# kritsanan1/Qwen3-TTS

Measured on AMD Instinct MI355X. Metric: audio-seconds/sec (RTF) + p50 first-packet latency, 1.7B @ batch 1/8, 1->8 GPU, higher is better.
Workload: dtype bf16; 1 GPU; Qwen3-TTS-12Hz-1.7b-customvoice B=8/GPU x 200-token prompts, streaming text, 256 frames + codec decode; global_batch=8, seq_len=200, frames=256, parallelism=dp1

## Files before the change

### qwen3-tts_amd/csrc/codec_unit.hip

```cpp
#include "common.h"

namespace {

constexpr int CU_TAPS = 7;
constexpr int CU_MAX_DIL = 9;

constexpr int unit_wpe(int C, int MI) { return C == 96 ? (MI == 4 ? 2 : 4) : (MI == 1 ? 3 : 2); }

template <int C, int MI>
__global__ __launch_bounds__(256) __attribute__((amdgpu_waves_per_eu(unit_wpe(C, MI)))) void codec_unit_k(
    qt_codec_resunit_args p) {
  constexpr int BM = 64 * MI;
  constexpr int RT = BM / 32;
  constexpr int NCH = C / 32;
  constexpr int CT = C / 32;
  constexpr int G = C / 8;
  constexpr int LDW = C + 8;
  constexpr int RPI = 256 / G;
  constexpr int NR = BM * G / 256;
  static_assert(BM * G % 256 == 0, "output tile groups divide over the block");
  extern __shared__ __attribute__((aligned(16))) unsigned char cu_smem[];
  bf16_t* img = (bf16_t*)cu_smem;
  const int tid = threadIdx.x, lane = tid & 63, w = tid >> 6;
  const int lm = lane & 15, lk = lane >> 4;
  const int dil = p.dil, halo = (CU_TAPS - 1) * dil, WR = BM + halo;
  const int tiles_t = (p.L + BM - 1) / BM;
  const int bi = blockIdx.x / tiles_t, t0 = (blockIdx.x - bi * tiles_t) * BM;
  const bf16_t* xin = (const bf16_t*)p.x_in + (long long)bi * p.L * C;
  bf16_t* xout = (bf16_t*)p.x_out + (long long)bi * p.L * C;

  {
    const int g = tid % G, r0 = tid / G;
    if (r0 < RPI) {
      float sa[8], sib[8];
      load8f(p.s1_alpha + g * 8, sa);
      load8f(p.s1_inv_beta + g * 8, sib);
      for (int rb = r0; rb < WR; rb += 4 * RPI) {
        u32x4_t raw[4];
#pragma unroll
        for (int u = 0; u < 4; ++u) {
          const int r = rb + u * RPI, ti = t0 - halo + r;
          raw[u] = u32x4_t{0u, 0u, 0u, 0u};
          if (r < WR && ti >= 0 && ti < p.L) raw[u] = *(const u32x4_t*)(xin + (long long)ti * C + g * 8);
        }
#pragma unroll
        for (int u = 0; u < 4; ++u) {
          const int r = rb + u * RPI;
          if (r >= WR) break;
          float v[8];
#pragma unroll
          for (int i = 0; i < 4; ++i) {
            v[2 * i] = __uint_as_float(raw[u][i] << 16);
            v[2 * i + 1] = __uint_as_float(raw[u][i] & 0xFFFF0000u);
          }
#pragma unroll
          for (int e = 0; e < 8; ++e) {
            const float sn = __sinf(v[e] * sa[e]);
            v[e] = v[e] + sib[e] * (sn * sn);
          }
          *(u32x4_t*)(img + r * LDW + g * 8) =
              u32x4_t{pack2bf(v[0], v[1]), pack2bf(v[2], v[3]), pack2bf(v[4], v[5]), pack2bf(v[6], v[7])};
        }
      }
    }
  }

  const int wrow = (w >> 1) * (BM / 2);
  const int nt0 = (w & 1) * CT;
  f32x4_t acc[RT][CT];
#pragma unroll
  for (int i = 0; i < RT; ++i)
#pragma unroll
    for (int q = 0; q < CT; ++q) acc[i][q] = f32x4_t{0.f, 0.f, 0.f, 0.f};

  {
    constexpr int KT = CU_TAPS * NCH;
    const bf16_t* Wb = (const bf16_t*)p.w1 + lane * 8;
    u32x4_t cur[CT], nxt[CT];
#pragma unroll
    for (int q = 0; q < CT; ++q) cur[q] = *(const u32x4_t*)(Wb + ((size_t)(nt0 + q) * KT) * 512);
    __syncthreads();
#pragma unroll 1
    for (int c = 0; c < NCH; ++c) {
      const bf16_t* wa = img + (wrow + lm) * LDW + c * 32 + lk * 8;
#pragma unroll
      for (int j = 0; j < CU_TAPS; ++j) {
        const int kn = j + 1 < CU_TAPS ? (j + 1) * NCH + c : (c + 1 < NCH ? c + 1 : c);
#pragma unroll
        for (int q = 0; q < CT; ++q) nxt[q] = *(const u32x4_t*)(Wb + ((size_t)(nt0 + q) * KT + kn) * 512);
        u32x4_t af[RT];
#pragma unroll
        for (int i = 0; i < RT; ++i) af[i] = *(const u32x4_t*)(wa + (i * 16 + j * dil) * LDW);
#pragma unroll
        for (int i = 0; i < RT; ++i)
#pragma unroll
          for (int q = 0; q < CT; ++q)
            acc[i][q] = __builtin_amdgcn_mfma_f32_16x16x32_bf16(__builtin_bit_cast(bf16x8_t, af[i]),
                                                                __builtin_bit_cast(bf16x8_t, cur[q]), acc[i][q], 0, 0, 0);
#pragma unroll
        for (int q = 0; q < CT; ++q) cur[q] = nxt[q];
      }
    }
  }
  __syncthreads();

  u32x4_t xr[NR];
#pragma unroll
  for (int u = 0; u < NR; ++u) {
    const int q = tid + u * 256, r = q / G, g = q - r * G;
    xr[u] = u32x4_t{0u, 0u, 0u, 0u};
    if (t0 + r < p.L) xr[u] = *(const u32x4_t*)(xin + (long long)(t0 + r) * C + g * 8);
  }

#pragma unroll
  for (int q = 0; q < CT; ++q) {
    const int n = (nt0 + q) * 16 + lm;
    const float b1 = p.b1 ? p.b1[n] : 0.f, a2 = p.s2_alpha[n], ib2 = p.s2_inv_beta[n];
#pragma unroll
    for (int i = 0; i < RT; ++i)
#pragma unroll
      for (int e = 0; e < 4; ++e) {
        const float h = bf2f(f2bf(acc[i][q][e] + b1));
        const float sn = __sinf(h * a2);
        img[(wrow + i * 16 + lk * 4 + e) * LDW + n] = f2bf(h + ib2 * (sn * sn));
        acc[i][q][e] = 0.f;
      }
  }

  {
    const bf16_t* Wb = (const bf16_t*)p.w2 + lane * 8;
    u32x4_t cur[CT], nxt[CT];
#pragma unroll
    for (int q = 0; q < CT; ++q) cur[q] = *(const u32x4_t*)(Wb + ((size_t)(nt0 + q) * NCH) * 512);
    __syncthreads();
    const bf16_t* wa = img + (wrow + lm) * LDW + lk * 8;
#pragma unroll
    for (int c = 0; c < NCH; ++c) {
      const int kn = c + 1 < NCH ? c + 1 : c;
#pragma unroll
      for (int q = 0; q < CT; ++q) nxt[q] = *(const u32x4_t*)(Wb + ((size_t)(nt0 + q) * NCH + kn) * 512);
      u32x4_t af[RT];
#pragma unroll
      for (int i = 0; i < RT; ++i) af[i] = *(const u32x4_t*)(wa + i * 16 * LDW + c * 32);
#pragma unroll
      for (int i = 0; i < RT; ++i)
#pragma unroll
        for (int q = 0; q < CT; ++q)
          acc[i][q] = __builtin_amdgcn_mfma_f32_16x16x32_bf16(__builtin_bit_cast(bf16x8_t, af[i]),
                                                              __builtin_bit_cast(bf16x8_t, cur[q]), acc[i][q], 0, 0, 0);
#pragma unroll
      for (int q = 0; q < CT; ++q) cur[q] = nxt[q];
    }
  }
  __syncthreads();

#pragma unroll
  for (int u = 0; u < NR; ++u) {
    const int q = tid + u * 256, r = q / G, g = q - r * G;
    *(u32x4_t*)(img + r * LDW + g * 8) = xr[u];
  }
  __syncthreads();
#pragma unroll
  for (int q = 0; q < CT; ++q) {
    const int n = (nt0 + q) * 16 + lm;
    const float b2 = p.b2 ? p.b2[n] : 0.f;
#pragma unroll
    for (int i = 0; i < RT; ++i)
#pragma unroll
      for (int e = 0; e < 4; ++e) {
        bf16_t* s = img + (wrow + i * 16 + lk * 4 + e) * LDW + n;
        *s = f2bf(bf2f(*s) + (acc[i][q][e] + b2));
      }
  }
  __syncthreads();

#pragma unroll
  for (int u = 0; u < NR; ++u) {
    const int q = tid + u * 256, r = q / G, g = q - r * G;
    if (t0 + r < p.L) *(u32x4_t*)(xout + (long long)(t0 + r) * C + g * 8) = *(const u32x4_t*)(img + r * LDW + g * 8);
  }
}

size_t unit_smem(int C, int bm, int dil) { return (size_t)(bm + (CU_TAPS - 1) * dil) * (C + 8) * sizeof(bf16_t); }

template <int C, int MI>
int launch_unit(const qt_codec_resunit_args& a, hipStream_t s) {
  constexpr int BM = 64 * MI;
  const size_t smem = unit_smem(C, BM, a.dil);
  if (smem > (64u << 10) &&
      hipFuncSetAttribute((const void*)codec_unit_k<C, MI>, hipFuncAttributeMaxDynamicSharedMemorySize,
                          (int)unit_smem(C, BM, CU_MAX_DIL)) != hipSuccess)
    return QT_ERR_LAUNCH;
  const long long blocks = (long long)a.B * ((a.L + BM - 1) / BM);
  hipLaunchKernelGGL((codec_unit_k<C, MI>), dim3((unsigned)blocks), dim3(256), smem, s, a);
  return hipGetLastError() == hipSuccess ? QT_OK : QT_ERR_LAUNCH;
}

}

static int unit_check(const qt_codec_resunit_args* a) {
  if (!a) return QT_ERR_ARG;
  if (a->a_dtype != QT_BF16 || a->w_dtype != QT_BF16) return QT_ERR_DTYPE;
  if (a->C != 96 && a->C != 192) return QT_ERR_SHAPE;
  if (a->dil != 1 && a->dil != 3 && a->dil != CU_MAX_DIL) return QT_ERR_SHAPE;
  if (a->B < 1 || a->L < 1 || (long long)a->B * ((a->L + 63) / 64) > 0x7FFFFFFFLL) return QT_ERR_SHAPE;
  if (!a->x_in || !a->x_out || !a->w1 || !a->w2 || !a->s1_alpha || !a->s1_inv_beta || !a->s2_alpha || !a->s2_inv_beta)
    return QT_ERR_ARG;
  if ((reinterpret_cast<uintptr_t>(a->x_in) | reinterpret_cast<uintptr_t>(a->x_out) | reinterpret_cast<uintptr_t>(a->w1) |
       reinterpret_cast<uintptr_t>(a->w2) | reinterpret_cast<uintptr_t>(a->s1_alpha) |
       reinterpret_cast<uintptr_t>(a->s1_inv_beta)) & 15)
    return QT_ERR_ARG;
  const unsigned long long bytes = (unsigned long long)a->B * a->L * a->C * sizeof(bf16_t);
  const uintptr_t xi = reinterpret_cast<uintptr_t>(a->x_in), xo = reinterpret_cast<uintptr_t>(a->x_out);
  if (xi < xo + bytes && xo < xi + bytes) return QT_ERR_ARG;
  return QT_OK;
}

extern "C" int qt_codec_resunit_supported(const qt_codec_resunit_args* a) { return unit_check(a) == QT_OK; }

extern "C" int qt_codec_resunit(const qt_codec_resunit_args* a, void* stream) {
  const int rc = unit_check(a);
  if (rc != QT_OK) return rc;
  hipStream_t s = (hipStream_t)stream;
  if constexpr (kProbe) {
    const int mi = qt_knob("QT_CU_MI", 0);
    if (a->C == 96 && mi == 1) return launch_unit<96, 1>(*a, s);
    if (a->C == 96 && mi == 4) return launch_unit<96, 4>(*a, s);
    if (a->C == 192 && (mi == 2 || mi == 4)) return launch_unit<192, 2>(*a, s);
  }
  if (a->C == 96) return launch_unit<96, 2>(*a, s);
  return launch_unit<192, 1>(*a, s);
}
```

Before: 251.4 audio-seconds/sec.

## Add fused wide-channel codec residual-unit kernel for C=384/768

Adds a new fused residual-unit kernel for codec decoder stages with 384 or 768 channels, which were previously rejected by the shape check and so fell back to another path. Input channels are streamed through a double-buffered shared-memory window in KC-sized chunks, with the snake activation applied on the fly, so the dilated 7-tap conv, the second snake, the 1x1 conv and the residual add all run in one kernel. This targets the separate launches and global-memory round trips the unfused path needs. In exchange it adds a large templated kernel with probe knobs and many MFMA accumulators per wave, which may increase register pressure.

```diff
diff --git a/qwen3-tts_amd/csrc/codec_unit.hip b/qwen3-tts_amd/csrc/codec_unit.hip
--- a/qwen3-tts_amd/csrc/codec_unit.hip
+++ b/qwen3-tts_amd/csrc/codec_unit.hip
@@ -196,12 +196,226 @@
   return hipGetLastError() == hipSuccess ? QT_OK : QT_ERR_LAUNCH;
 }
 
+constexpr int wide_threads(int C) { return 128 * (C / 96); }
+constexpr int WIDE_KC = 64, WIDE_RT = 4;
+
+constexpr size_t wide_img_bytes(int C, int KC, int dil) {
+  const size_t win = (size_t)2 * (64 + (CU_TAPS - 1) * dil) * (KC + 8) * sizeof(bf16_t);
+  const size_t at = (size_t)64 * (C + 8) * sizeof(bf16_t);
+  return win > at ? win : at;
+}
+constexpr size_t wide_smem(int C, int KC, int dil) { return wide_img_bytes(C, KC, dil) + (size_t)2 * C * sizeof(float); }
+
+template <int C, int KC, int RT>
+__global__ __launch_bounds__(wide_threads(C)) __attribute__((amdgpu_waves_per_eu(4))) void codec_unit_wide_k(
+    qt_codec_resunit_args p) {
+  constexpr int BM = 64;
+  constexpr int CT = 12 / RT;
+  constexpr int NTH = wide_threads(C);
+  constexpr int NWC = C / (16 * CT);
+  constexpr int NCH = C / 32;
+  constexpr int SUB = KC / 32;
+  constexpr int NCC = C / KC;
+  constexpr int G = C / 8;
+  constexpr int GK = KC / 8;
+  constexpr int LDW = C + 8;
+  constexpr int LDK = KC + 8;
+  constexpr int RPI = NTH / GK;
+  constexpr int NP = (BM + (CU_TAPS - 1) * CU_MAX_DIL + RPI - 1) / RPI;
+  constexpr int NR = BM * G / NTH;
+  static_assert((RT == 2 || RT == 4) && C % 96 == 0 && C % KC == 0 && KC % 32 == 0 && NTH % GK == 0 && BM * G % NTH == 0, "wide unit geometry");
+  extern __shared__ __attribute__((aligned(16))) unsigned char cu_smem[];
+  const int tid = threadIdx.x, lane = tid & 63, w = tid >> 6;
+  const int lm = lane & 15, lk = lane >> 4;
+  const int dil = p.dil, halo = (CU_TAPS - 1) * dil, WR = BM + halo;
+  bf16_t* img = (bf16_t*)cu_smem;
+  float* sn1 = (float*)(cu_smem + wide_img_bytes(C, KC, dil));
+  const int tiles_t = (p.L + BM - 1) / BM;
+  const int bi = blockIdx.x / tiles_t, t0 = (blockIdx.x - bi * tiles_t) * BM;
+  const bf16_t* xin = (const bf16_t*)p.x_in + (long long)bi * p.L * C;
+  bf16_t* xout = (bf16_t*)p.x_out + (long long)bi * p.L * C;
+
+  const int sg = tid % GK, sr0 = tid / GK;
+  u32x4_t raw[NP];
+  auto load_chunk = [&](int cc) {
+#pragma unroll
+    for (int u = 0; u < NP; ++u) {
+      const int r = sr0 + u * RPI, ti = t0 - halo + r;
+      raw[u] = u32x4_t{0u, 0u, 0u, 0u};
+      if (r < WR && ti >= 0 && ti < p.L) raw[u] = *(const u32x4_t*)(xin + (long long)ti * C + cc * KC + sg * 8);
+    }
+  };
+  auto store_chunk = [&](int buf, int cc) {
+    bf16_t* wb = img + (size_t)buf * WR * LDK;
+    float sa[8], sib[8];
+    load8f(sn1 + cc * KC + sg * 8, sa);
+    load8f(sn1 + C + cc * KC + sg * 8, sib);
+#pragma unroll
+    for (int u = 0; u < NP; ++u) {
+      const int r = sr0 + u * RPI;
+      if (r >= WR) break;
+      float v[8];
+#pragma unroll
+      for (int i = 0; i < 4; ++i) {
+        v[2 * i] = __uint_as_float(raw[u][i] << 16);
+        v[2 * i + 1] = __uint_as_float(raw[u][i] & 0xFFFF0000u);
+      }
+#pragma unroll
+      for (int e = 0; e < 8; ++e) {
+        const float sn = __sinf(v[e] * sa[e]);
+        v[e] = v[e] + sib[e] * (sn * sn);
+      }
+      *(u32x4_t*)(wb + r * LDK + sg * 8) =
+          u32x4_t{pack2bf(v[0], v[1]), pack2bf(v[2], v[3]), pack2bf(v[4], v[5]), pack2bf(v[6], v[7])};
+    }
+  };
+
+  load_chunk(0);
+  for (int i = tid; i < C; i += NTH) {
+    sn1[i] = p.s1_alpha[i];
+    sn1[C + i] = p.s1_inv_beta[i];
+  }
+  __syncthreads();
+  store_chunk(0, 0);
+
+  const int wrow = (w / NWC) * (16 * RT);
+  const int nt0 = (w % NWC) * CT;
+  f32x4_t acc[RT][CT];
+#pragma unroll
+  for (int i = 0; i < RT; ++i)
+#pragma unroll
+    for (int q = 0; q < CT; ++q) acc[i][q] = f32x4_t{0.f, 0.f, 0.f, 0.f};
+
+  {
+    constexpr int KT = CU_TAPS * NCH;
+    const bf16_t* Wb = (const bf16_t*)p.w1 + lane * 8;
+    u32x4_t cur[CT], nxt[CT];
+#pragma unroll
+    for (int q = 0; q < CT; ++q) cur[q] = *(const u32x4_t*)(Wb + ((size_t)(nt0 + q) * KT) * 512);
+    __syncthreads();
+#pragma unroll 1
+    for (int c = 0; c < NCH; ++c) {
+      const int cc = c / SUB, sub = c - cc * SUB;
+      if (sub == 0 && cc + 1 < NCC) load_chunk(cc + 1);
+      const bf16_t* wa = img + (size_t)(cc & 1) * WR * LDK + (wrow + lm) * LDK + sub * 32 + lk * 8;
+#pragma unroll
+      for (int j = 0; j < CU_TAPS; ++j) {
+        const int kn = j + 1 < CU_TAPS ? (j + 1) * NCH + c : (c + 1 < NCH ? c + 1 : c);
+#pragma unroll
+        for (int q = 0; q < CT; ++q) nxt[q] = *(const u32x4_t*)(Wb + ((size_t)(nt0 + q) * KT + kn) * 512);
+        u32x4_t af[RT];
+#pragma unroll
+        for (int i = 0; i < RT; ++i) af[i] = *(const u32x4_t*)(wa + (i * 16 + j * dil) * LDK);
+#pragma unroll
+        for (int i = 0; i < RT; ++i)
+#pragma unroll
+          for (int q = 0; q < CT; ++q)
+            acc[i][q] = __builtin_amdgcn_mfma_f32_16x16x32_bf16(__builtin_bit_cast(bf16x8_t, af[i]),
+                                                                __builtin_bit_cast(bf16x8_t, cur[q]), acc[i][q], 0, 0, 0);
+#pragma unroll
+        for (int q = 0; q < CT; ++q) cur[q] = nxt[q];
+      }
+      if (sub == SUB - 1) {
+        if (cc + 1 < NCC) store_chunk((cc + 1) & 1, cc + 1);
+        __syncthreads();
+      }
+    }
+  }
+
+#pragma unroll
+  for (int q = 0; q < CT; ++q) {
+    const int n = (nt0 + q) * 16 + lm;
+    const float b1 = p.b1 ? p.b1[n] : 0.f, a2 = p.s2_alpha[n], ib2 = p.s2_inv_beta[n];
+#pragma unroll
+    for (int i = 0; i < RT; ++i)
+#pragma unroll
+      for (int e = 0; e < 4; ++e) {
+        const float h = bf2f(f2bf(acc[i][q][e] + b1));
+        const float sn = __sinf(h * a2);
+        img[(wrow + i * 16 + lk * 4 + e) * LDW + n] = f2bf(h + ib2 * (sn * sn));
+        acc[i][q][e] = 0.f;
+      }
+  }
+
+  {
+    const bf16_t* Wb = (const bf16_t*)p.w2 + lane * 8;
+    u32x4_t cur[CT], nxt[CT];
+#pragma unroll
+    for (int q = 0; q < CT; ++q) cur[q] = *(const u32x4_t*)(Wb + ((size_t)(nt0 + q) * NCH) * 512);
+    __syncthreads();
+    const bf16_t* wa = img + (wrow + lm) * LDW + lk * 8;
+#pragma unroll 2
+    for (int c = 0; c < NCH; ++c) {
+      const int kn = c + 1 < NCH ? c + 1 : c;
+#pragma unroll
+      for (int q = 0; q < CT; ++q) nxt[q] = *(const u32x4_t*)(Wb + ((size_t)(nt0 + q) * NCH + kn) * 512);
+      u32x4_t af[RT];
+#pragma unroll
+      for (int i = 0; i < RT; ++i) af[i] = *(const u32x4_t*)(wa + i * 16 * LDW + c * 32);
+#pragma unroll
+      for (int i = 0; i < RT; ++i)
+#pragma unroll
+        for (int q = 0; q < CT; ++q)
+          acc[i][q] = __builtin_amdgcn_mfma_f32_16x16x32_bf16(__builtin_bit_cast(bf16x8_t, af[i]),
+                                                              __builtin_bit_cast(bf16x8_t, cur[q]), acc[i][q], 0, 0, 0);
+#pragma unroll
+      for (int q = 0; q < CT; ++q) cur[q] = nxt[q];
+    }
+  }
+
+  u32x4_t xr[NR];
+#pragma unroll
+  for (int u = 0; u < NR; ++u) {
+    const int q = tid + u * NTH, r = q / G, g = q - r * G;
+    xr[u] = u32x4_t{0u, 0u, 0u, 0u};
+    if (t0 + r < p.L) xr[u] = *(const u32x4_t*)(xin + (long long)(t0 + r) * C + g * 8);
+  }
+  __syncthreads();
+#pragma unroll
+  for (int u = 0; u < NR; ++u) {
+    const int q = tid + u * NTH, r = q / G, g = q - r * G;
+    *(u32x4_t*)(img + r * LDW + g * 8) = xr[u];
+  }
+  __syncthreads();
+#pragma unroll
+  for (int q = 0; q < CT; ++q) {
+    const int n = (nt0 + q) * 16 + lm;
+    const float b2 = p.b2 ? p.b2[n] : 0.f;
+#pragma unroll
+    for (int i = 0; i < RT; ++i)
+#pragma unroll
+      for (int e = 0; e < 4; ++e) {
+        bf16_t* s = img + (wrow + i * 16 + lk * 4 + e) * LDW + n;
+        *s = f2bf(bf2f(*s) + (acc[i][q][e] + b2));
+      }
+  }
+  __syncthreads();
+
+#pragma unroll
+  for (int u = 0; u < NR; ++u) {
+    const int q = tid + u * NTH, r = q / G, g = q - r * G;
+    if (t0 + r < p.L) *(u32x4_t*)(xout + (long long)(t0 + r) * C + g * 8) = *(const u32x4_t*)(img + r * LDW + g * 8);
+  }
+}
+
+template <int C, int KC, int RT>
+int launch_wide(const qt_codec_resunit_args& a, hipStream_t s) {
+  const size_t smem = wide_smem(C, KC, a.dil);
+  if (smem > (64u << 10) &&
+      hipFuncSetAttribute((const void*)codec_unit_wide_k<C, KC, RT>, hipFuncAttributeMaxDynamicSharedMemorySize,
+                          (int)wide_smem(C, KC, CU_MAX_DIL)) != hipSuccess)
+    return QT_ERR_LAUNCH;
+  const long long blocks = (long long)a.B * ((a.L + 63) / 64);
+  hipLaunchKernelGGL((codec_unit_wide_k<C, KC, RT>), dim3((unsigned)blocks), dim3(wide_threads(C)), smem, s, a);
+  return hipGetLastError() == hipSuccess ? QT_OK : QT_ERR_LAUNCH;
+}
+
 }
 
 static int unit_check(const qt_codec_resunit_args* a) {
   if (!a) return QT_ERR_ARG;
   if (a->a_dtype != QT_BF16 || a->w_dtype != QT_BF16) return QT_ERR_DTYPE;
-  if (a->C != 96 && a->C != 192) return QT_ERR_SHAPE;
+  if (a->C != 96 && a->C != 192 && a->C != 384 && a->C != 768) return QT_ERR_SHAPE;
   if (a->dil != 1 && a->dil != 3 && a->dil != CU_MAX_DIL) return QT_ERR_SHAPE;
   if (a->B < 1 || a->L < 1 || (long long)a->B * ((a->L + 63) / 64) > 0x7FFFFFFFLL) return QT_ERR_SHAPE;
   if (!a->x_in || !a->x_out || !a->w1 || !a->w2 || !a->s1_alpha || !a->s1_inv_beta || !a->s2_alpha || !a->s2_inv_beta)
@@ -228,6 +442,27 @@
     if (a->C == 96 && mi == 4) return launch_unit<96, 4>(*a, s);
     if (a->C == 192 && (mi == 2 || mi == 4)) return launch_unit<192, 2>(*a, s);
   }
+  if constexpr (kProbe) {
+    const int kc = qt_knob("QT_CU_KC", 0), rt = qt_knob("QT_CU_RT", 0);
+    if (a->C == 384 || a->C == 768) {
+      const int v = (a->C == 768) * 1000 + (kc ? kc : WIDE_KC) * 4 + (rt ? rt : WIDE_RT);
+      switch (v) {
+        case 32 * 4 + 2: return launch_wide<384, 32, 2>(*a, s);
+        case 64 * 4 + 2: return launch_wide<384, 64, 2>(*a, s);
+        case 128 * 4 + 2: return launch_wide<384, 128, 2>(*a, s);
+        case 32 * 4 + 4: return launch_wide<384, 32, 4>(*a, s);
+        case 64 * 4 + 4: return launch_wide<384, 64, 4>(*a, s);
+        case 1000 + 32 * 4 + 2: return launch_wide<768, 32, 2>(*a, s);
+        case 1000 + 64 * 4 + 2: return launch_wide<768, 64, 2>(*a, s);
+        case 1000 + 128 * 4 + 2: return launch_wide<768, 128, 2>(*a, s);
+        case 1000 + 32 * 4 + 4: return launch_wide<768, 32, 4>(*a, s);
+        case 1000 + 64 * 4 + 4: return launch_wide<768, 64, 4>(*a, s);
+        default: return QT_ERR_ARG;
+      }
+    }
+  }
+  if (a->C == 384) return launch_wide<384, WIDE_KC, WIDE_RT>(*a, s);
+  if (a->C == 768) return launch_wide<768, WIDE_KC, WIDE_RT>(*a, s);
   if (a->C == 96) return launch_unit<96, 2>(*a, s);
   return launch_unit<192, 1>(*a, s);
 }
```

After: 252.3 audio-seconds/sec, median of 4. Within noise of the previous version (+0.4%).
